# Artemarius/cuda-gaussian-splatting

Hardware: AMD Instinct MI355X
Metric: fwd+bwd Mpixels/s @1080p, 1M Gaussians, SH3 (higher is better)
Workload: dtype f32

## Files before the change

### cuda-gaussian-splatting_amd/csrc/cugs_raster_common.h

```cpp
#pragma once

#include "cugs_gaussian_math.h"

#define CUGS_REC_F4 3

struct RasterGeom {
    int width, height, ntx, ntiles;
    float bg0, bg1, bg2;
};

struct RasterSrc {
    const int32_t* tile_ranges;
    const int32_t* gidx;
    const float* packed;
    const float* means_2d;
    const float* cov_2d_inv;
    const float* rgb;
    const float* opa;
    const uint4* tile_order;
};

template <bool PACKED, bool DEPTH = false>
__device__ __forceinline__ int stage_record(const RasterSrc& s, int li, int end, float4* s_rec,
                                            const float* __restrict__ depths = nullptr) {
    if (li >= end) return -1;
    const int g = s.gidx[li];
    float4 r0, r1, r2;
    if (PACKED) {
        const float4* src = reinterpret_cast<const float4*>(s.packed + (int64_t)g * CUGS_PACKED_STRIDE);
        r0 = src[0]; r1 = src[1]; r2 = src[2];
    } else {
        const float a = s.cov_2d_inv[g * 3 + 0], c = s.cov_2d_inv[g * 3 + 2], o = s.opa[g];
        r0 = make_float4(s.means_2d[g * 2 + 0], s.means_2d[g * 2 + 1], a, s.cov_2d_inv[g * 3 + 1]);
        r1 = make_float4(c, o, (o >= (1.0f / 255.0f)) ? logf(255.0f * o) : -1.0f, 0.0f);
        r2 = make_float4(s.rgb[g * 3 + 0], 0.0f, s.rgb[g * 3 + 1], s.rgb[g * 3 + 2]);
    }
    r1.w = __int_as_float(g);
    if (DEPTH) r2.y = depths[g];
    s_rec[threadIdx.x * CUGS_REC_F4 + 0] = r0;
    s_rec[threadIdx.x * CUGS_REC_F4 + 1] = r1;
    s_rec[threadIdx.x * CUGS_REC_F4 + 2] = r2;
    return g;
}

__device__ __forceinline__ bool may_touch_quad(float4 r0, float4 r1, float qx0, float qy0,
                                               float wx, float wy) {
    const float mx = r0.x, my = r0.y, a = r0.z, b = r0.w, c = r1.x;
    const float tau = r1.z;
    if (!(tau >= 0.0f)) return false;
    if (!(a > 0.0f && c > 0.0f)) return true;
    const float ia = __builtin_amdgcn_rcpf(a), ic = __builtin_amdgcn_rcpf(c);
    const float lx = qx0 - mx, hx = lx + wx, ly = qy0 - my, hy = ly + wy;
    const bool inside = (lx <= 0.0f) && (hx >= 0.0f) && (ly <= 0.0f) && (hy >= 0.0f);
    float X, Y;
    asm("v_max_f32_e64 %0, -%1, %2" : "=v"(X) : "v"(lx), "v"(hx));
    asm("v_max_f32_e64 %0, -%1, %2" : "=v"(Y) : "v"(ly), "v"(hy));
    const float B = a * X * X + 2.0f * fabsf(b) * X * Y + c * Y * Y;
    const float b2 = b + b;
    const float xe = (lx > 0.0f) ? lx : hx, ye = (ly > 0.0f) ? ly : hy;
    const float yv = __builtin_amdgcn_fmed3f(-b * xe * ic, ly, hy);
    const float xv = __builtin_amdgcn_fmed3f(-b * ye * ia, lx, hx);
    const float qx = a * xe * xe + b2 * xe * yv + c * yv * yv;
    const float qy = a * xv * xv + b2 * xv * ye + c * ye * ye;
    const bool out_x = !((lx <= 0.0f) && (hx >= 0.0f)), out_y = !((ly <= 0.0f) && (hy >= 0.0f));
    const float qmin = inside ? 0.0f : fminf(out_x ? qx : 3.0e38f, out_y ? qy : 3.0e38f);
    return !(0.5f * qmin > tau * 1.01f + 0.05f + 4e-6f * B);
}

struct ActiveRect { float x0, y0, wx, wy; };
__device__ __forceinline__ ActiveRect active_rect(unsigned long long active, float quad_cx, float quad_cy) {
    unsigned cols = (unsigned)active | (unsigned)(active >> 32);
    cols |= cols >> 16;
    cols |= cols >> 8;
    cols &= 0xFFu;
    const int x0 = __builtin_ctz(cols), x1 = 31 - __builtin_clz(cols);
    const int y0 = __builtin_ctzll(active) >> 3, y1 = (63 - __builtin_clzll(active)) >> 3;
    return ActiveRect{quad_cx + (float)x0, quad_cy + (float)y0, (float)(x1 - x0), (float)(y1 - y0)};
}

#define CUGS_HIT_GROUP 4
__device__ __forceinline__ unsigned cugs_pop_hit_desc(unsigned long long& mask) {
    const unsigned bit = 63u - (unsigned)__builtin_clzll(mask);
    mask &= ~(1ull << bit);
    return bit;
}
__device__ __forceinline__ unsigned cugs_pop_hit_asc(unsigned long long& mask) {
    const unsigned bit = (unsigned)__builtin_ctzll(mask);
    mask &= mask - 1ull;
    return bit;
}
__device__ __forceinline__ unsigned long long cugs_pop_hits4_desc(unsigned long long& mask, unsigned rec_base) {
    const unsigned r0 = rec_base + cugs_pop_hit_desc(mask) * CUGS_REC_F4;
    const unsigned r1 = rec_base + cugs_pop_hit_desc(mask) * CUGS_REC_F4;
    const unsigned r2 = rec_base + cugs_pop_hit_desc(mask) * CUGS_REC_F4;
    const unsigned r3 = rec_base + cugs_pop_hit_desc(mask) * CUGS_REC_F4;
    return (unsigned long long)(r0 | (r1 << 16)) | ((unsigned long long)(r2 | (r3 << 16)) << 32);
}
__device__ __forceinline__ int cugs_hit(unsigned long long hitrecs, int field) {
    return (int)((hitrecs >> (16 * field)) & 0xFFFFull);
}
__device__ __forceinline__ unsigned long long cugs_set_hit(unsigned long long hitrecs, int field, unsigned rec) {
    return (hitrecs & ~(0xFFFFull << (16 * field))) | ((unsigned long long)rec << (16 * field));
}

struct PixelEval { float dx, dy, gx, gy, e; };
__device__ __forceinline__ float pixel_alpha_raw(float pxf, float pyf, float mx, float my, float a, float b,
                                                 float c, float o, float open, PixelEval& r) {
    r.dx = pxf - mx;
    r.dy = pyf - my;
    r.gx = fmaf(a, r.dx, b * r.dy);
    r.gy = fmaf(b, r.dx, c * r.dy);
    const float q = fmaf(r.dx, r.gx, r.dy * r.gy);
    r.e = cugs_blend_exp_q(q);
    const float gate = fmaf(q, 0x1p127f, 1.0f);
    return __builtin_fminf(__builtin_fminf((o * open) * r.e, 0.99f), gate);
}
__device__ __forceinline__ float pixel_alpha(float pxf, float pyf, float mx, float my, float a, float b,
                                             float c, float o, float open, PixelEval& r) {
    const float alpha = pixel_alpha_raw(pxf, pyf, mx, my, a, b, c, o, open, r);
    return (alpha < (1.0f / 255.0f)) ? 0.0f : alpha;
}


__device__ __forceinline__ float sat_fma(float a, float b, float c) {
    return __builtin_amdgcn_fmed3f(fmaf(a, b, c), 0.0f, 1.0f);
}
__device__ __forceinline__ float sat_add(float a, float b) { return __builtin_amdgcn_fmed3f(a + b, 0.0f, 1.0f); }

#define CUGS_ALPHA_MIN_PRED 0x1.01010p-8f
__device__ __forceinline__ float passes_alpha_min(float x) {
    return sat_fma(x, 0x1p32f, -CUGS_ALPHA_MIN_PRED * 0x1p32f);
}
__device__ __forceinline__ float below_alpha_cap(float x) { return sat_fma(x, -0x1p32f, 0.99f * 0x1p32f); }

__device__ __forceinline__ int reduce9t_slot(int lane) {
    if (lane & 3) return -1;
    const int bank = (lane >> 2) & 3, row = lane >> 4;
    const int perm[4] = {0, 2, 1, 3};
    if (row == 0) return perm[bank];
    if (row == 1) return bank == 3 ? 8 : 4 + perm[bank];
    if (row == 2 && bank == 0) return 7;
    return -1;
}

__device__ __forceinline__ float reduce9t(float cA, float cB, float v2, float v3, float v4, float v5, float v6,
                                          float v8, float v7) {
    float a0, a1, a2, a3, a4, b0, b1, b2, d;
    asm volatile(
// ... 126 lines not shown
```

### cuda-gaussian-splatting_amd/csrc/raster_backward.hip

```cpp
#include "cugs_raster_common.h"

#include <cstdlib>

#ifdef CUGS_DEV
bool cugs_dev_backward_stats();
#endif

namespace {

#define CUGS_BWD_HITS 4
static_assert(CUGS_BWD_HITS == CUGS_HIT_GROUP, "a hit group is one flush");
#ifndef CUGS_BWD_HSTRIDE
#define CUGS_BWD_HSTRIDE 64
#endif

template <bool PACKED, bool WIDE, bool STATS, bool DEPTH = false>
__global__ __launch_bounds__(CUGS_BLOCK) __attribute__((amdgpu_waves_per_eu(DEPTH ? 7 : 8)))
void k_raster_backward(RasterGeom geo, RasterSrc src,
                                                                const float* __restrict__ dL_dcolor,
                                                                const float* __restrict__ final_T,
                                                                const int32_t* __restrict__ n_contrib,
                                                                float* __restrict__ grad_accum, int64_t stats_row,
                                                                const float* __restrict__ depths,
                                                                const float* __restrict__ dL_ddepth_map,
                                                                const float* __restrict__ dL_dalpha) {
    __shared__ float4 s_rec[CUGS_BLOCK * CUGS_REC_F4];
    __shared__ float2 s_contrib[4][CUGS_BWD_HITS][CUGS_BWD_HSTRIDE];

#ifdef CUGS_DEV
    const bool no_atomics = stats_row == -2;
#else
    constexpr bool no_atomics = false;
#endif
    unsigned tile;
    int range_start, range_end;
    if (src.tile_order) {
        const uint4 rec = src.tile_order[blockIdx.x];
        tile = rec.x; range_start = (int)rec.y; range_end = (int)rec.z;
    } else {
        tile = cugs_blend_tile(blockIdx.x, (unsigned)geo.ntx, (unsigned)(geo.ntiles / geo.ntx));
        range_start = src.tile_ranges[tile * 2 + 0];
        range_end = src.tile_ranges[tile * 2 + 1];
    }
    const int tile_x = (int)(tile % (unsigned)geo.ntx), tile_y = (int)(tile / (unsigned)geo.ntx);
    const int tid = threadIdx.x, wave = tid >> 6, lane = tid & 63;
    const int quad_x = tile_x * CUGS_TILE + (wave & 1) * 8, quad_y = tile_y * CUGS_TILE + (wave >> 1) * 8;
    const int px = quad_x + (lane & 7), py = quad_y + (lane >> 3);
    const bool inside = (px < geo.width) && (py < geo.height);
    const float pxf = (float)px + 0.5f, pyf = (float)py + 0.5f;
    const float qx0 = (float)quad_x + 0.5f, qy0 = (float)quad_y + 0.5f;

    const int num_in_range = range_end - range_start;
    const int num_batches = (num_in_range + CUGS_BLOCK - 1) / CUGS_BLOCK;

    const int pix = py * geo.width + px;
    float T = inside ? final_T[pix] : 0.0f;
    const int max_contrib = inside ? n_contrib[pix] : 0;
    float dC0 = 0.0f, dC1 = 0.0f, dC2 = 0.0f;
    if (inside) {
        dC0 = dL_dcolor[pix * 3 + 0];
        dC1 = dL_dcolor[pix * 3 + 1];
        dC2 = dL_dcolor[pix * 3 + 2];
    }
    float dDp = 0.0f;
    if (DEPTH && inside && dL_ddepth_map) dDp = dL_ddepth_map[pix];
    const int h2 = lane >> 4, g2i = lane & 15;
    const int gx0 = quad_x + (g2i & 1) * 4, gy = quad_y + (g2i >> 1);
    const float px2 = (float)gx0 + 0.5f, py2 = (float)gy + 0.5f;
    const bool side = (lane & 8) != 0;
    float eA[4], eB[4], e2[4], eZ[4];
#pragma unroll
    for (int i = 0; i < 4; ++i) {
        float r = 0.0f, gg = 0.0f, bb = 0.0f, zz = 0.0f;
        if (gx0 + i < geo.width && gy < geo.height) {
            const int pq = gy * geo.width + gx0 + i, q = pq * 3;
            r = dL_dcolor[q + 0]; gg = dL_dcolor[q + 1]; bb = dL_dcolor[q + 2];
            if (DEPTH && dL_ddepth_map) zz = dL_ddepth_map[pq];
        }
        eA[i] = side ? gg : r; eB[i] = side ? r : gg; e2[i] = bb; eZ[i] = zz;
    }
    const int slot2 = DEPTH ? reduce10r16_slot(lane) : reduce9r16_slot(lane);
    const unsigned slot_off = (unsigned)(slot2 < 0 ? 0 : slot2) * 4u;
    unsigned long long hitrecs = 0ull;

    float D = fmaf(dC2, T * geo.bg2, fmaf(dC1, T * geo.bg1, dC0 * (T * geo.bg0)));
    if (DEPTH && inside && dL_dalpha) D = fmaf(-T, dL_dalpha[pix], D);
    float rem = (inside && max_contrib > 0) ? (float)max_contrib : -1.0f;
    float open = (inside && max_contrib > 0) ? 1.0f : 0.0f;
    bool wave_done = (__ballot(open != 0.0f) == 0ull);
    int pending = 0;
    unsigned st_steps = 0, st_contrib = 0, st_lanes = 0, st_batches = 0, st_tested = 0, st_open = 0;

    auto flush = [&](int cnt) {
        const int rec = (int)((hitrecs >> (16 * h2)) & 0xFFFFull);
        const float4* c4 = reinterpret_cast<const float4*>(&s_contrib[wave][h2][g2i * 4]);
        const float4 p01 = c4[0], p23 = c4[1];
        const float2 mean = *reinterpret_cast<const float2*>(&s_rec[rec]);
        const float4 tail = s_rec[rec + 1];
        const float dy = py2 - mean.y;
        const float dx0 = px2 - mean.x, dx1 = dx0 + 1.0f, dx2 = dx0 + 2.0f, dx3 = dx0 + 3.0f;
        float t = p01.y * dx0;
        float A = p01.y, M1 = t, Mxx = t * dx0;
        float RA = p01.x * eA[0], RB = p01.x * eB[0], R2 = p01.x * e2[0];
        t = p01.w * dx1; A += p01.w; M1 += t; Mxx = fmaf(t, dx1, Mxx);
        RA = fmaf(p01.z, eA[1], RA); RB = fmaf(p01.z, eB[1], RB); R2 = fmaf(p01.z, e2[1], R2);
        t = p23.y * dx2; A += p23.y; M1 += t; Mxx = fmaf(t, dx2, Mxx);
        RA = fmaf(p23.x, eA[2], RA); RB = fmaf(p23.x, eB[2], RB); R2 = fmaf(p23.x, e2[2], R2);
        t = p23.w * dx3; A += p23.w; M1 += t; Mxx = fmaf(t, dx3, Mxx);
        RA = fmaf(p23.z, eA[3], RA); RB = fmaf(p23.z, eB[3], RB); R2 = fmaf(p23.z, e2[3], R2);
        const float oA = tail.y * A;
        M1 *= tail.y; Mxx *= tail.y;
        const float M1y = dy * oA, Myy = dy * M1y, Mxy = dy * M1;
        float total;
        if (DEPTH) {
            float RZ = p01.x * eZ[0];
            RZ = fmaf(p01.z, eZ[1], RZ); RZ = fmaf(p23.x, eZ[2], RZ); RZ = fmaf(p23.z, eZ[3], RZ);
            total = reduce10r16(RA, RB, R2, A, M1, M1y, Mxx, Myy, Mxy, RZ, lane);
        } else {
            total = reduce9r16(RA, RB, R2, A, M1, M1y, Mxx, Myy, Mxy, lane);
        }
        if (slot2 >= 0 && h2 < cnt && !no_atomics) {
            const int g = __float_as_int(tail.w);
            if (WIDE) {
                atomicAdd(grad_accum + (int64_t)g * CUGS_GRAD_STRIDE + slot2, total);
            } else {
                const unsigned off = ((unsigned)g << 6) + slot_off;
                atomicAdd(reinterpret_cast<float*>(reinterpret_cast<char*>(grad_accum) + off), total);
            }
        }
    };

    auto step = [&](const int rec, const int slot) __attribute__((always_inline)) {
        if (STATS) ++st_steps;
        const float4 g0 = s_rec[rec], g1 = s_rec[rec + 1], col = s_rec[rec + 2];
        const float o = g1.y;

        PixelEval e;
        const float alpha = pixel_alpha_raw(pxf, pyf, g0.x, g0.y, g0.z, g0.w, g1.x, o, open, e);
        const float passf = passes_alpha_min(alpha);
        rem -= passf;
        open = sat_add(rem, 1.0f);
        const float k = passf * open;
        const float al = alpha * k;
        const float gk = k * below_alpha_cap(alpha);

        const float rcp = __builtin_amdgcn_rcpf(1.0f - al);
        T *= rcp;
        const float weight = al * T;
        float G = fmaf(dC2, col.w, fmaf(dC1, col.z, dC0 * col.x));
        if (DEPTH) G = fmaf(dDp, col.y, G);
        const float gate = fmaf(T, G, -(rcp * D)) * gk;
        D = fmaf(weight, G, D);
        if (STATS) {
            const unsigned long long lm = __ballot(k != 0.0f);
            if (lm) { ++st_contrib; st_lanes += __popcll(lm); st_open += __popcll(__ballot(open != 0.0f)); }
        }
        s_contrib[wave][slot][lane] = make_float2(weight, gate * e.e);
    };

    for (int batch = num_batches - 1; batch >= 0; --batch) {
        if (lane == 0) s_contrib[wave][0][0].x = wave_done ? 1.0f : 0.0f;
        __syncthreads();
        if (s_contrib[0][0][0].x * s_contrib[1][0][0].x * s_contrib[2][0][0].x * s_contrib[3][0][0].x != 0.0f) break;

        stage_record<PACKED, DEPTH>(src, range_start + batch * CUGS_BLOCK + tid, range_end, s_rec, depths);
        __syncthreads();

        if (STATS && !wave_done) ++st_batches;
        if (!wave_done) {
            const int batch_count = min(CUGS_BLOCK, num_in_range - batch * CUGS_BLOCK);
            const int nsub = (batch_count + CUGS_WAVE - 1) / CUGS_WAVE;
            for (int sub = nsub - 1; sub >= 0 && !wave_done; --sub) {
                const int j = sub * CUGS_WAVE + lane;
                const ActiveRect ar = active_rect(__ballot(open != 0.0f), qx0, qy0);
                bool hit = false;
                if (j < batch_count)
                    hit = may_touch_quad(s_rec[j * CUGS_REC_F4 + 0], s_rec[j * CUGS_REC_F4 + 1], ar.x0, ar.y0, ar.wx,
                                         ar.wy);
                unsigned long long mask = __ballot(hit);
                if (STATS) st_tested += min(CUGS_WAVE, batch_count - sub * CUGS_WAVE);
                const unsigned rec_sub = (unsigned)(sub * CUGS_WAVE * CUGS_REC_F4);
                while (pending + __popcll(mask) >= CUGS_BWD_HITS) {
                    if (pending == 0) {
                        hitrecs = cugs_pop_hits4_desc(mask, rec_sub);
                    } else {
                        do hitrecs = cugs_set_hit(hitrecs, pending, rec_sub + cugs_pop_hit_desc(mask) * CUGS_REC_F4);
                        while (++pending < CUGS_BWD_HITS);
                        pending = 0;
                    }
                    step(cugs_hit(hitrecs, 0), 0);
                    step(cugs_hit(hitrecs, 1), 1);
                    step(cugs_hit(hitrecs, 2), 2);
                    step(cugs_hit(hitrecs, 3), 3);
                    const bool closed = (__ballot(open != 0.0f) == 0ull);
                    flush(CUGS_BWD_HITS);
                    if (closed) { wave_done = true; mask = 0ull; break; }
                }
                while (mask != 0ull) {
                    hitrecs = cugs_set_hit(hitrecs, pending, rec_sub + cugs_pop_hit_desc(mask) * CUGS_REC_F4);
                    ++pending;
                }
            }
            if (pending) {
                for (int p = 0; p < pending; ++p) step(cugs_hit(hitrecs, p), p);
                if (__ballot(open != 0.0f) == 0ull) wave_done = true;
                flush(pending);
                pending = 0;
            }
        }
    }
    if (STATS && lane == 0) {
        float* st = grad_accum + (int64_t)stats_row * CUGS_GRAD_STRIDE;
        atomicAdd(&st[0], (float)st_steps); atomicAdd(&st[1], (float)st_contrib); atomicAdd(&st[2], (float)st_lanes);
        atomicAdd(&st[3], (float)st_batches); atomicAdd(&st[4], (float)st_tested); atomicAdd(&st[5], (float)num_batches);
        atomicAdd(&st[7], (float)st_open);
    }
}

template <bool PACKED, bool DEPTH = false>
__global__ __launch_bounds__(CUGS_BLOCK) void k_unpack_grads(int64_t n, const float* __restrict__ acc,
                                                             const float* __restrict__ packed,
                                                             const float* __restrict__ cov_2d_inv,
                                                             float* __restrict__ dL_drgb,
                                                             float* __restrict__ dL_dopa,
                                                             float* __restrict__ dL_dmeans,
                                                             float* __restrict__ dL_dcov,
                                                             float* __restrict__ dL_ddepths) {
    const int64_t i = (int64_t)blockIdx.x * CUGS_BLOCK + threadIdx.x;
    if (i >= n) return;
    const float4* row = reinterpret_cast<const float4*>(acc + i * CUGS_GRAD_STRIDE);
    const float4 r0 = row[0], r1 = row[1];
    float r2;
    if (DEPTH) {
        const float2 w89 = *reinterpret_cast<const float2*>(acc + i * CUGS_GRAD_STRIDE + 8);
        r2 = w89.x;
        dL_ddepths[i] = w89.y;
    } else {
        r2 = acc[i * CUGS_GRAD_STRIDE + 8];
    }
    float a, b, c;
    if (PACKED) {
        const float4* rec = reinterpret_cast<const float4*>(packed + i * CUGS_PACKED_STRIDE);
        const float4 p0 = rec[0];
        a = p0.z; b = p0.w; c = rec[1].x;
    } else {
        a = cov_2d_inv[i * 3 + 0]; b = cov_2d_inv[i * 3 + 1]; c = cov_2d_inv[i * 3 + 2];
    }
    dL_drgb[i * 3 + 0] = r0.x; dL_drgb[i * 3 + 1] = r0.y; dL_drgb[i * 3 + 2] = r0.z;
    dL_dopa[i] = r0.w;
    const GradMoments m{r1.x, r1.y, r1.z, r1.w, r2};
    const Grad2D g = grads_from_moments(m, a, b, c);
    dL_dmeans[i * 2 + 0] = g.mx; dL_dmeans[i * 2 + 1] = g.my;
    dL_dcov[i * 3 + 0] = g.a; dL_dcov[i * 3 + 1] = g.b; dL_dcov[i * 3 + 2] = g.c;
}

}

namespace {
int rasterize_backward_impl(int width, int height, const float background_host[3],
                                       const int32_t* tile_ranges, const int32_t* gaussian_indices,
                                       const float* means_2d, const float* cov_2d_inv, const float* rgb,
                                       const float* opacities_act, const float* packed,
                                       const float* dL_dcolor, const float* final_T,
                                       const int32_t* n_contrib, int64_t n, float* grad_accum,
                                       float* dL_drgb, float* dL_dopacity_act, float* dL_dmeans_2d,
                                       float* dL_dcov_2d_inv, bool prezeroed, const uint32_t* tile_order, void* stream,
                                       bool depth_map = false, const float* depths = nullptr,
                                       const float* dL_ddepth_map = nullptr, const float* dL_dalpha = nullptr,
// ... 142 lines not shown
                      in[6 * 64 + l], in[8 * 64 + l], in[7 * 64 + l]);
    slots[l] = reduce9t_slot(l);
}
__global__ void k_dbg_reduce9r16(const float* __restrict__ in, float* __restrict__ out, int* __restrict__ slots) {
    const int l = threadIdx.x;
    const bool side = (l & 8) != 0;
    const float v0 = in[0 * 64 + l], v1 = in[1 * 64 + l];
    out[l] = reduce9r16(side ? v1 : v0, side ? v0 : v1, in[2 * 64 + l], in[3 * 64 + l], in[4 * 64 + l], in[5 * 64 + l],
                        in[6 * 64 + l], in[8 * 64 + l], in[7 * 64 + l], l);
    slots[l] = reduce9r16_slot(l);
}
__global__ void k_dbg_reduce10r16(const float* __restrict__ in, float* __restrict__ out, int* __restrict__ slots) {
    const int l = threadIdx.x;
    const bool side = (l & 8) != 0;
    const float v0 = in[0 * 64 + l], v1 = in[1 * 64 + l];
    out[l] = reduce10r16(side ? v1 : v0, side ? v0 : v1, in[2 * 64 + l], in[3 * 64 + l], in[4 * 64 + l], in[5 * 64 + l],
                         in[6 * 64 + l], in[8 * 64 + l], in[7 * 64 + l], in[9 * 64 + l], l);
    slots[l] = reduce10r16_slot(l);
}
__global__ void k_dbg_rcp(const float* __restrict__ in, float* __restrict__ out, int n) {
    const int i = blockIdx.x * blockDim.x + threadIdx.x;
    if (i < n) out[i] = __builtin_amdgcn_rcpf(in[i]);
}
__global__ void k_dbg_blend_exp(const float* __restrict__ q, float* __restrict__ out, int n) {
    const int i = blockIdx.x * blockDim.x + threadIdx.x;
    if (i < n) out[i] = cugs_blend_exp_q(q[i]);
}
__global__ void k_dbg_may_touch_quad(int n, const float* __restrict__ in, const unsigned long long* __restrict__ masks,
                                     int* __restrict__ hit, unsigned long long* __restrict__ pass,
                                     float* __restrict__ rect) {
    const int i = blockIdx.x * blockDim.x + threadIdx.x;
    if (i >= n) return;
    const float* c = in + (int64_t)i * 8;
    alignas(16) float rec[CUGS_PACKED_STRIDE];
    write_packed(rec, 0, c[0], c[1], Sym2{c[2], c[3], c[4]}, 0.0f, 0.0f, 0.0f, c[5]);
    const float4 r0 = reinterpret_cast<const float4*>(rec)[0], r1 = reinterpret_cast<const float4*>(rec)[1];
    const int quad_x = (int)c[6], quad_y = (int)c[7];
    const float qx0 = (float)quad_x + 0.5f, qy0 = (float)quad_y + 0.5f;
    const unsigned long long active = masks[i];
    const ActiveRect ar = active_rect(active, qx0, qy0);
    hit[i] = may_touch_quad(r0, r1, ar.x0, ar.y0, ar.wx, ar.wy) ? 1 : 0;
    unsigned long long p = 0ull;
    for (int l = 0; l < 64; ++l) {
        const float pxf = (float)(quad_x + (l & 7)) + 0.5f, pyf = (float)(quad_y + (l >> 3)) + 0.5f;
        const float open = ((active >> l) & 1ull) ? 1.0f : 0.0f;
        PixelEval e;
        const float alpha = pixel_alpha_raw(pxf, pyf, r0.x, r0.y, r0.z, r0.w, r1.x, r1.y, open, e);
        if (passes_alpha_min(alpha) != 0.0f) p |= 1ull << l;
    }
    pass[i] = p;
    rect[(int64_t)i * 4 + 0] = ar.x0 - qx0; rect[(int64_t)i * 4 + 1] = ar.y0 - qy0;
    rect[(int64_t)i * 4 + 2] = ar.wx; rect[(int64_t)i * 4 + 3] = ar.wy;
}
bool g_dev_backward_stats = false;
}
bool cugs_dev_backward_stats() { return g_dev_backward_stats; }
extern "C" int cugsdbg_backward_stats(int on) { g_dev_backward_stats = (on != 0); return 0; }
extern "C" int cugsdbg_reduce9(const float* in, float* out, int* slots, void* stream) {
    hipLaunchKernelGGL(k_dbg_reduce9, dim3(1), dim3(64), 0, static_cast<hipStream_t>(stream), in, out, slots);
    CUGS_LAUNCH_CHECK();
    return 0;
}
extern "C" int cugsdbg_reduce9r16(const float* in, float* out, int* slots, void* stream) {
    hipLaunchKernelGGL(k_dbg_reduce9r16, dim3(1), dim3(64), 0, static_cast<hipStream_t>(stream), in, out, slots);
    CUGS_LAUNCH_CHECK();
    return 0;
}
extern "C" int cugsdbg_reduce10r16(const float* in, float* out, int* slots, void* stream) {
    hipLaunchKernelGGL(k_dbg_reduce10r16, dim3(1), dim3(64), 0, static_cast<hipStream_t>(stream), in, out, slots);
    CUGS_LAUNCH_CHECK();
    return 0;
}
extern "C" int cugsdbg_blend_exp_q(const float* q, float* out, int n, void* stream) {
    hipLaunchKernelGGL(k_dbg_blend_exp, dim3((n + 255) / 256), dim3(256), 0, static_cast<hipStream_t>(stream), q, out, n);
    CUGS_LAUNCH_CHECK();
    return 0;
}
extern "C" int cugsdbg_rcp(const float* in, float* out, int n, void* stream) {
    hipLaunchKernelGGL(k_dbg_rcp, dim3((n + 255) / 256), dim3(256), 0, static_cast<hipStream_t>(stream), in, out, n);
    CUGS_LAUNCH_CHECK();
    return 0;
}
extern "C" int cugsdbg_may_touch_quad(int n, const float* in, const unsigned long long* masks, int* hit,
                                      unsigned long long* pass, float* rect, void* stream) {
    if (n <= 0) return n == 0 ? 0 : CUGS_EINVAL;
    hipLaunchKernelGGL(k_dbg_may_touch_quad, dim3((n + 255) / 256), dim3(256), 0, static_cast<hipStream_t>(stream), n, in,
                       masks, hit, pass, rect);
    CUGS_LAUNCH_CHECK();
    return 0;
}
#endif
```

### cuda-gaussian-splatting_amd/csrc/raster_forward.hip

```cpp
#include "cugs_raster_common.h"

namespace {

template <bool PACKED, bool DEPTH>
__device__ __forceinline__ void raster_forward_tile(RasterGeom geo, RasterSrc src, float* out_color, float* out_final_T,
                                                    int32_t* out_n_contrib, float4* zero_buf, uint32_t zero_vec4,
                                                    const float* depths, float* out_depth) {
    __shared__ float4 s_rec[CUGS_BLOCK * CUGS_REC_F4];
    __shared__ int s_wave_done[4];

    if (zero_buf) {
        const uint32_t per = (zero_vec4 + gridDim.x - 1) / gridDim.x;
        const uint32_t lo = blockIdx.x * per, hi = min(zero_vec4, lo + per);
        for (uint32_t e = lo + threadIdx.x; e < hi; e += CUGS_BLOCK) cugs_stnt(zero_buf + e, make_float4(0.0f, 0.0f, 0.0f, 0.0f));
    }

    unsigned tile;
    int range_start, range_end;
    if (src.tile_order) {
        const uint4 rec = src.tile_order[blockIdx.x];
        tile = rec.x; range_start = (int)rec.y; range_end = (int)rec.z;
    } else {
        tile = cugs_blend_tile(blockIdx.x, (unsigned)geo.ntx, (unsigned)(geo.ntiles / geo.ntx));
        range_start = src.tile_ranges[tile * 2 + 0];
        range_end = src.tile_ranges[tile * 2 + 1];
    }
    const int tile_x = (int)(tile % (unsigned)geo.ntx), tile_y = (int)(tile / (unsigned)geo.ntx);
    const int tid = threadIdx.x, wave = tid >> 6, lane = tid & 63;
    const int quad_x = tile_x * CUGS_TILE + (wave & 1) * 8, quad_y = tile_y * CUGS_TILE + (wave >> 1) * 8;
    const int px = quad_x + (lane & 7), py = quad_y + (lane >> 3);
    const bool inside = (px < geo.width) && (py < geo.height);
    const float pxf = (float)px + 0.5f, pyf = (float)py + 0.5f;
    const float qx0 = (float)quad_x + 0.5f, qy0 = (float)quad_y + 0.5f;

    const int num_in_range = range_end - range_start;
    const int num_batches = (num_in_range + CUGS_BLOCK - 1) / CUGS_BLOCK;

    typedef float v2f __attribute__((ext_vector_type(2)));
    float T = 1.0f, C0 = 0.0f;
    v2f C12 = {0.0f, 0.0f};
    v2f C0Z = {0.0f, 0.0f};
    float count = 0.0f;
    float open = inside ? 1.0f : 0.0f;
    bool wave_done = (__ballot(open != 0.0f) == 0ull);

    auto step = [&](const float4* rp) __attribute__((always_inline)) {
        const float4 g0 = rp[0], g1 = rp[1], col = rp[2];
        const float o = g1.y;
        PixelEval e;
        const float alpha = pixel_alpha_raw(pxf, pyf, g0.x, g0.y, g0.z, g0.w, g1.x, o, open, e);
        const float passf = passes_alpha_min(alpha);
        const float al = alpha * passf;
        const float weight = al * T;
        if (DEPTH) C0Z = __builtin_elementwise_fma((v2f){weight, weight}, (v2f){col.x, col.y}, C0Z);
        else C0 = fmaf(weight, col.x, C0);
        C12 = __builtin_elementwise_fma((v2f){weight, weight}, (v2f){col.z, col.w}, C12);
        T *= (1.0f - al);
        count += passf;
        open *= passes_alpha_min(T);
    };

    for (int batch = 0; batch < num_batches; ++batch) {
        if (lane == 0) s_wave_done[wave] = wave_done ? 1 : 0;
        __syncthreads();
        if (s_wave_done[0] & s_wave_done[1] & s_wave_done[2] & s_wave_done[3]) break;

        stage_record<PACKED, DEPTH>(src, range_start + batch * CUGS_BLOCK + tid, range_end, s_rec, depths);
        __syncthreads();

        if (!wave_done) {
            const int batch_count = min(CUGS_BLOCK, num_in_range - batch * CUGS_BLOCK);
            for (int sub = 0; sub * CUGS_WAVE < batch_count && !wave_done; ++sub) {
                const int j = sub * CUGS_WAVE + lane;
                const ActiveRect ar = active_rect(__ballot(open != 0.0f), qx0, qy0);
                bool hit = false;
                if (j < batch_count)
                    hit = may_touch_quad(s_rec[j * CUGS_REC_F4 + 0], s_rec[j * CUGS_REC_F4 + 1], ar.x0, ar.y0, ar.wx,
                                         ar.wy);
                unsigned long long mask = __ballot(hit);
                const float4* sub_rec = s_rec + sub * CUGS_WAVE * CUGS_REC_F4;
                while (__popcll(mask) >= CUGS_HIT_GROUP) {
                    const float4* r0 = sub_rec + cugs_pop_hit_asc(mask) * CUGS_REC_F4;
                    const float4* r1 = sub_rec + cugs_pop_hit_asc(mask) * CUGS_REC_F4;
                    const float4* r2 = sub_rec + cugs_pop_hit_asc(mask) * CUGS_REC_F4;
                    const float4* r3 = sub_rec + cugs_pop_hit_asc(mask) * CUGS_REC_F4;
                    step(r0); step(r1); step(r2); step(r3);
                    if (__ballot(open != 0.0f) == 0ull) { wave_done = true; mask = 0ull; break; }
                }
                while (mask != 0ull) {
                    step(sub_rec + cugs_pop_hit_asc(mask) * CUGS_REC_F4);
                    if (__ballot(open != 0.0f) == 0ull) { wave_done = true; break; }
                }
            }
        }
    }

    if (inside) {
        const int pix = py * geo.width + px;
        if (DEPTH) {
            C0 = C0Z.x;
            out_depth[pix] = fmaf(T, 0.0f, C0Z.y);
        }
        out_color[pix * 3 + 0] = fmaf(T, geo.bg0, C0);
        out_color[pix * 3 + 1] = fmaf(T, geo.bg1, C12.x);
        out_color[pix * 3 + 2] = fmaf(T, geo.bg2, C12.y);
        out_final_T[pix] = T;
        out_n_contrib[pix] = (int)count;
    }
}

template <bool PACKED>
__global__ __launch_bounds__(CUGS_BLOCK) void k_raster_forward(RasterGeom geo, RasterSrc src,
                                                               float* __restrict__ out_color,
                                                               float* __restrict__ out_final_T,
                                                               int32_t* __restrict__ out_n_contrib,
                                                               float4* __restrict__ zero_buf, uint32_t zero_vec4) {
    raster_forward_tile<PACKED, false>(geo, src, out_color, out_final_T, out_n_contrib, zero_buf, zero_vec4, nullptr,
                                       nullptr);
}

template <bool PACKED>
__global__ __launch_bounds__(CUGS_BLOCK) void k_raster_forward_depth(RasterGeom geo, RasterSrc src,
                                                                     float* __restrict__ out_color,
                                                                     float* __restrict__ out_final_T,
                                                                     int32_t* __restrict__ out_n_contrib,
                                                                     float4* __restrict__ zero_buf, uint32_t zero_vec4,
                                                                     const float* __restrict__ depths,
                                                                     float* __restrict__ out_depth) {
    raster_forward_tile<PACKED, true>(geo, src, out_color, out_final_T, out_n_contrib, zero_buf, zero_vec4, depths,
                                      out_depth);
}

}

namespace {
int rasterize_forward_impl(int width, int height, const float background_host[3], const int32_t* tile_ranges,
                           const int32_t* gaussian_indices, const float* means_2d, const float* cov_2d_inv,
                           const float* rgb, const float* opacities_act, const float* packed, float* out_color,
                           float* out_final_T, int32_t* out_n_contrib, void* zero_buf, size_t zero_bytes,
                           const uint32_t* tile_order, void* stream, bool depth_map = false,
                           const float* depths = nullptr, float* out_depth = nullptr) {
    if (width < 0 || height < 0 || !background_host) return CUGS_EINVAL;
    if (zero_bytes && (!zero_buf || (reinterpret_cast<uintptr_t>(zero_buf) & 15u) || (zero_bytes & 15u) ||
                       zero_bytes / 16 > 0xFFFFFFFFull))
        return zero_buf ? CUGS_EALIGN : CUGS_EINVAL;
    const int ntx = (width + CUGS_TILE - 1) / CUGS_TILE, nty = (height + CUGS_TILE - 1) / CUGS_TILE;
    if (ntx == 0 || nty == 0) {
        if (zero_bytes) CUGS_RETURN_IF_HIP(hipMemsetAsync(zero_buf, 0, zero_bytes, static_cast<hipStream_t>(stream)));
        return 0;
// ... 19 lines not shown
    } else if (packed) {
        hipLaunchKernelGGL((k_raster_forward<true>), dim3(geo.ntiles), dim3(CUGS_BLOCK), 0, st, geo, src,
                           out_color, out_final_T, out_n_contrib, zb, zv);
    } else {
        hipLaunchKernelGGL((k_raster_forward<false>), dim3(geo.ntiles), dim3(CUGS_BLOCK), 0, st, geo, src,
                           out_color, out_final_T, out_n_contrib, zb, zv);
    }
    CUGS_LAUNCH_CHECK();
    return 0;
}
}

extern "C" int cugs_rasterize_forward(int width, int height, const float background_host[3],
                                      const int32_t* tile_ranges, const int32_t* gaussian_indices,
                                      const float* means_2d, const float* cov_2d_inv, const float* rgb,
                                      const float* opacities_act, const float* packed, float* out_color,
                                      float* out_final_T, int32_t* out_n_contrib, void* stream) {
    return rasterize_forward_impl(width, height, background_host, tile_ranges, gaussian_indices, means_2d, cov_2d_inv, rgb,
                                  opacities_act, packed, out_color, out_final_T, out_n_contrib, nullptr, 0, nullptr, stream);
}

extern "C" int cugs_rasterize_forward_zero(int width, int height, const float background_host[3],
                                           const int32_t* tile_ranges, const int32_t* gaussian_indices,
                                           const float* means_2d, const float* cov_2d_inv, const float* rgb,
                                           const float* opacities_act, const float* packed, float* out_color,
                                           float* out_final_T, int32_t* out_n_contrib, void* zero_buf,
                                           size_t zero_bytes, void* stream) {
    return rasterize_forward_impl(width, height, background_host, tile_ranges, gaussian_indices, means_2d, cov_2d_inv, rgb,
                                  opacities_act, packed, out_color, out_final_T, out_n_contrib, zero_buf, zero_bytes, nullptr, stream);
}

extern "C" int cugs_rasterize_forward_ordered(int width, int height, const float background_host[3],
                                              const int32_t* tile_ranges, const int32_t* gaussian_indices,
                                              const float* means_2d, const float* cov_2d_inv, const float* rgb,
                                              const float* opacities_act, const float* packed, float* out_color,
                                              float* out_final_T, int32_t* out_n_contrib, void* zero_buf,
                                              size_t zero_bytes, const uint32_t* tile_order, void* stream) {
    return rasterize_forward_impl(width, height, background_host, tile_ranges, gaussian_indices, means_2d, cov_2d_inv, rgb,
                                  opacities_act, packed, out_color, out_final_T, out_n_contrib, zero_buf, zero_bytes, tile_order,
                                  stream);
}

extern "C" int cugs_rasterize_forward_depth(int width, int height, const float background_host[3],
                                            const int32_t* tile_ranges, const int32_t* gaussian_indices,
                                            const float* means_2d, const float* cov_2d_inv, const float* rgb,
                                            const float* opacities_act, const float* packed, float* out_color,
                                            float* out_final_T, int32_t* out_n_contrib, void* zero_buf,
                                            size_t zero_bytes, const uint32_t* tile_order, const float* depths,
                                            float* out_depth, void* stream) {
    return rasterize_forward_impl(width, height, background_host, tile_ranges, gaussian_indices, means_2d, cov_2d_inv, rgb,
                                  opacities_act, packed, out_color, out_final_T, out_n_contrib, zero_buf, zero_bytes, tile_order,
                                  stream, true, depths, out_depth);
}
```

Baseline: 2705.

## Merge disjoint-coverage Gaussian pairs into single evaluation step in backward raster

While staging records, the backward kernel now computes a per-tile row/column coverage bitmask for each Gaussian and stores it in a spare record field. Two consecutive hits whose masks do not overlap within the wave's 8x8 quad are treated as twins. Each lane evaluates only the Gaussian that covers it and writes zero contributions for the other slot, so one eval replaces two. The cost is extra work per staged record, a bpermute and ballot per sub-batch, and more branching, and it only runs in the non-depth path.

```diff
diff --git a/cuda-gaussian-splatting_amd/csrc/cugs_raster_common.h b/cuda-gaussian-splatting_amd/csrc/cugs_raster_common.h
--- a/cuda-gaussian-splatting_amd/csrc/cugs_raster_common.h
+++ b/cuda-gaussian-splatting_amd/csrc/cugs_raster_common.h
@@ -20,9 +20,11 @@
     const uint4* tile_order;
 };
 
-template <bool PACKED, bool DEPTH = false>
+__device__ __forceinline__ unsigned cugs_tile_cover(float4 r0, float4 r1, float tcx0, float tcy0);
+template <bool PACKED, bool DEPTH = false, bool COVER = false>
 __device__ __forceinline__ int stage_record(const RasterSrc& s, int li, int end, float4* s_rec,
-                                            const float* __restrict__ depths = nullptr) {
+                                            const float* __restrict__ depths = nullptr, float tcx0 = 0.0f,
+                                            float tcy0 = 0.0f) {
     if (li >= end) return -1;
     const int g = s.gidx[li];
     float4 r0, r1, r2;
@@ -37,6 +39,7 @@
     }
     r1.w = __int_as_float(g);
     if (DEPTH) r2.y = depths[g];
+    if (COVER && !DEPTH) r2.y = __uint_as_float(cugs_tile_cover(r0, r1, tcx0, tcy0));
     s_rec[threadIdx.x * CUGS_REC_F4 + 0] = r0;
     s_rec[threadIdx.x * CUGS_REC_F4 + 1] = r1;
     s_rec[threadIdx.x * CUGS_REC_F4 + 2] = r2;
@@ -78,6 +81,50 @@
     return ActiveRect{quad_cx + (float)x0, quad_cy + (float)y0, (float)(x1 - x0), (float)(y1 - y0)};
 }
 
+#define CUGS_COVER_FULL 0xFFFFFFFFu
+__device__ __forceinline__ unsigned cugs_cover_bits(float lo, float ext) {
+    const float f0 = fminf(fmaxf(ceilf(-lo - ext), 0.0f), 16.0f), f1 = fminf(fmaxf(floorf(ext - lo), -1.0f), 15.0f);
+    if (!(f0 <= f1)) return (lo != lo || ext != ext) ? 0xFFFFu : 0u;
+    return (2u << (unsigned)(int)f1) - (1u << (unsigned)(int)f0);
+}
+__device__ __forceinline__ unsigned cugs_tile_cover(float4 r0, float4 r1, float tcx0, float tcy0) {
+    const float mx = r0.x, my = r0.y, a = r0.z, b = r0.w, c = r1.x, tau = r1.z;
+    const float ac = a * c, det = ac - b * b;
+    if (!(tau >= 0.0f && a > 0.0f && c > 0.0f && det > ac * 0x1p-10f)) return CUGS_COVER_FULL;
+    const float lx = tcx0 - mx, ly = tcy0 - my;
+    const float X = fmaxf(-lx, lx + 15.0f), Y = fmaxf(-ly, ly + 15.0f);
+    const float B = a * X * X + 2.0f * fabsf(b) * X * Y + c * Y * Y;
+    const float r = 2.0f * (tau * 1.01f + 0.05f + 4e-6f * B) / det;
+    return cugs_cover_bits(lx, sqrtf(r * c)) | (cugs_cover_bits(ly, sqrtf(r * a)) << 16);
+}
+__device__ __forceinline__ unsigned cugs_quad_cover(int wave) {
+    return (0xFFu << (8 * (wave & 1))) | (0xFF0000u << (8 * (wave >> 1)));
+}
+__device__ __forceinline__ bool cugs_covers_meet(unsigned cov_a, unsigned cov_b, unsigned quad) {
+    const unsigned t = cov_a & cov_b & quad;
+    return (t & 0xFFFFu) != 0u && (t >> 16) != 0u;
+}
+__device__ __forceinline__ unsigned long long cugs_cover_lanes(unsigned cov, int wave) {
+    const unsigned cols = (cov >> (8 * (wave & 1))) & 0xFFu, rows = (cov >> (16 + 8 * (wave >> 1))) & 0xFFu;
+    if (rows == 0u) return 0ull;
+    const unsigned y0 = (unsigned)__builtin_ctz(rows), n = (unsigned)__builtin_popcount(rows);
+    const unsigned long long run = (n >= 8u) ? ~0ull : (((1ull << (8u * n)) - 1ull) << (8u * y0));
+    const unsigned c4 = cols * 0x01010101u;
+    return run & (((unsigned long long)c4 << 32) | c4);
+}
+__device__ __forceinline__ int cugs_select_lanes(int a, int b, unsigned long long m) {
+    int r;
+    asm("v_cndmask_b32_e64 %0, %1, %2, %3" : "=v"(r) : "v"(a), "v"(b), "s"(m));
+    return r;
+}
+__device__ __forceinline__ unsigned long long cugs_twin_mask(unsigned long long mask, bool hit, unsigned cov,
+                                                              unsigned quad, int lane) {
+    const unsigned long long above = (mask >> 1) >> lane;
+    const int prev = (lane + 1 + __builtin_ctzll(above | (1ull << 63))) & 63;
+    const unsigned pc = (unsigned)__builtin_amdgcn_ds_bpermute(prev << 2, (int)cov);
+    return __ballot(hit && above != 0ull && !cugs_covers_meet(cov, pc, quad));
+}
+
 #define CUGS_HIT_GROUP 4
 __device__ __forceinline__ unsigned cugs_pop_hit_desc(unsigned long long& mask) {
     const unsigned bit = 63u - (unsigned)__builtin_clzll(mask);
@@ -94,6 +141,16 @@
     const unsigned r1 = rec_base + cugs_pop_hit_desc(mask) * CUGS_REC_F4;
     const unsigned r2 = rec_base + cugs_pop_hit_desc(mask) * CUGS_REC_F4;
     const unsigned r3 = rec_base + cugs_pop_hit_desc(mask) * CUGS_REC_F4;
+    return (unsigned long long)(r0 | (r1 << 16)) | ((unsigned long long)(r2 | (r3 << 16)) << 32);
+}
+__device__ __forceinline__ unsigned long long cugs_pop_hits4_desc_twins(unsigned long long& mask, unsigned rec_base,
+                                                                        unsigned long long twins, unsigned& tw) {
+    const unsigned b0 = cugs_pop_hit_desc(mask), b1 = cugs_pop_hit_desc(mask), b2 = cugs_pop_hit_desc(mask),
+                   b3 = cugs_pop_hit_desc(mask);
+    tw = (unsigned)((twins >> b1) & 1ull) | ((unsigned)((twins >> b2) & 1ull) << 1) |
+         ((unsigned)((twins >> b3) & 1ull) << 2);
+    const unsigned r0 = rec_base + b0 * CUGS_REC_F4, r1 = rec_base + b1 * CUGS_REC_F4;
+    const unsigned r2 = rec_base + b2 * CUGS_REC_F4, r3 = rec_base + b3 * CUGS_REC_F4;
     return (unsigned long long)(r0 | (r1 << 16)) | ((unsigned long long)(r2 | (r3 << 16)) << 32);
 }
 __device__ __forceinline__ int cugs_hit(unsigned long long hitrecs, int field) {
diff --git a/cuda-gaussian-splatting_amd/csrc/raster_backward.hip b/cuda-gaussian-splatting_amd/csrc/raster_backward.hip
--- a/cuda-gaussian-splatting_amd/csrc/raster_backward.hip
+++ b/cuda-gaussian-splatting_amd/csrc/raster_backward.hip
@@ -26,6 +26,7 @@
                                                                 const float* __restrict__ dL_dalpha) {
     __shared__ float4 s_rec[CUGS_BLOCK * CUGS_REC_F4];
     __shared__ float2 s_contrib[4][CUGS_BWD_HITS][CUGS_BWD_HSTRIDE];
+    constexpr bool TWIN = !DEPTH;
 
 #ifdef CUGS_DEV
     const bool no_atomics = stats_row == -2;
@@ -49,6 +50,9 @@
     const bool inside = (px < geo.width) && (py < geo.height);
     const float pxf = (float)px + 0.5f, pyf = (float)py + 0.5f;
     const float qx0 = (float)quad_x + 0.5f, qy0 = (float)quad_y + 0.5f;
+    const float tcx0 = (float)(tile_x * CUGS_TILE) + 0.5f, tcy0 = (float)(tile_y * CUGS_TILE) + 0.5f;
+    const int wave_s = __builtin_amdgcn_readfirstlane(wave);
+    const unsigned quad_cover = cugs_quad_cover(wave_s);
 
     const int num_in_range = range_end - range_start;
     const int num_batches = (num_in_range + CUGS_BLOCK - 1) / CUGS_BLOCK;
@@ -89,7 +93,7 @@
     float open = (inside && max_contrib > 0) ? 1.0f : 0.0f;
     bool wave_done = (__ballot(open != 0.0f) == 0ull);
     int pending = 0;
-    unsigned st_steps = 0, st_contrib = 0, st_lanes = 0, st_batches = 0, st_tested = 0, st_open = 0;
+    unsigned st_steps = 0, st_contrib = 0, st_lanes = 0, st_batches = 0, st_tested = 0, st_open = 0, st_twins = 0;
 
     auto flush = [&](int cnt) {
         const int rec = (int)((hitrecs >> (16 * h2)) & 0xFFFFull);
@@ -130,9 +134,8 @@
         }
     };
 
-    auto step = [&](const int rec, const int slot) __attribute__((always_inline)) {
+    auto eval = [&](const float4 g0, const float4 g1, const float4 col) __attribute__((always_inline)) {
         if (STATS) ++st_steps;
-        const float4 g0 = s_rec[rec], g1 = s_rec[rec + 1], col = s_rec[rec + 2];
         const float o = g1.y;
 
         PixelEval e;
@@ -155,7 +158,20 @@
             const unsigned long long lm = __ballot(k != 0.0f);
             if (lm) { ++st_contrib; st_lanes += __popcll(lm); st_open += __popcll(__ballot(open != 0.0f)); }
         }
-        s_contrib[wave][slot][lane] = make_float2(weight, gate * e.e);
+        return make_float2(weight, gate * e.e);
+    };
+    auto step = [&](const int rec, const int slot) __attribute__((always_inline)) {
+        s_contrib[wave][slot][lane] = eval(s_rec[rec], s_rec[rec + 1], s_rec[rec + 2]);
+    };
+    auto twin = [&](const int rec_a, const int rec_b, const int slot_a, const int slot_b) __attribute__((always_inline)) {
+        if (STATS) ++st_twins;
+        const unsigned cov_b = (unsigned)__builtin_amdgcn_readfirstlane((int)__float_as_uint(s_rec[rec_b + 2].y));
+        const unsigned long long in_b = cugs_cover_lanes(cov_b, wave_s);
+        const int rec = cugs_select_lanes(rec_a, rec_b, in_b);
+        const float2 v = eval(s_rec[rec], s_rec[rec + 1], s_rec[rec + 2]);
+        const int slot = cugs_select_lanes(slot_a, slot_b, in_b);
+        s_contrib[wave][slot][lane] = v;
+        s_contrib[wave][slot_a + slot_b - slot][lane] = make_float2(0.0f, 0.0f);
     };
 
     for (int batch = num_batches - 1; batch >= 0; --batch) {
@@ -163,7 +179,7 @@
         __syncthreads();
         if (s_contrib[0][0][0].x * s_contrib[1][0][0].x * s_contrib[2][0][0].x * s_contrib[3][0][0].x != 0.0f) break;
 
-        stage_record<PACKED, DEPTH>(src, range_start + batch * CUGS_BLOCK + tid, range_end, s_rec, depths);
+        stage_record<PACKED, DEPTH, TWIN>(src, range_start + batch * CUGS_BLOCK + tid, range_end, s_rec, depths, tcx0, tcy0);
         __syncthreads();
 
         if (STATS && !wave_done) ++st_batches;
@@ -180,18 +196,35 @@
                 unsigned long long mask = __ballot(hit);
                 if (STATS) st_tested += min(CUGS_WAVE, batch_count - sub * CUGS_WAVE);
                 const unsigned rec_sub = (unsigned)(sub * CUGS_WAVE * CUGS_REC_F4);
+                unsigned long long twins = 0ull;
+                if (TWIN && pending + __popcll(mask) >= CUGS_BWD_HITS)
+                    twins = cugs_twin_mask(mask, hit, __float_as_uint(s_rec[(j & (CUGS_BLOCK - 1)) * CUGS_REC_F4 + 2].y),
+                                           quad_cover, lane);
                 while (pending + __popcll(mask) >= CUGS_BWD_HITS) {
+                    unsigned tw = 0u;
                     if (pending == 0) {
-                        hitrecs = cugs_pop_hits4_desc(mask, rec_sub);
+                        if (TWIN) hitrecs = cugs_pop_hits4_desc_twins(mask, rec_sub, twins, tw);
+                        else hitrecs = cugs_pop_hits4_desc(mask, rec_sub);
                     } else {
                         do hitrecs = cugs_set_hit(hitrecs, pending, rec_sub + cugs_pop_hit_desc(mask) * CUGS_REC_F4);
                         while (++pending < CUGS_BWD_HITS);
                         pending = 0;
                     }
-                    step(cugs_hit(hitrecs, 0), 0);
-                    step(cugs_hit(hitrecs, 1), 1);
-                    step(cugs_hit(hitrecs, 2), 2);
-                    step(cugs_hit(hitrecs, 3), 3);
+                    if (!TWIN || tw == 0u) {
+                        step(cugs_hit(hitrecs, 0), 0);
+                        step(cugs_hit(hitrecs, 1), 1);
+                        step(cugs_hit(hitrecs, 2), 2);
+                        step(cugs_hit(hitrecs, 3), 3);
+                    } else if ((tw & 5u) == 0u) {
+                        step(cugs_hit(hitrecs, 0), 0);
+                        twin(cugs_hit(hitrecs, 1), cugs_hit(hitrecs, 2), 1, 2);
+                        step(cugs_hit(hitrecs, 3), 3);
+                    } else {
+                        if (tw & 1u) twin(cugs_hit(hitrecs, 0), cugs_hit(hitrecs, 1), 0, 1);
+                        else { step(cugs_hit(hitrecs, 0), 0); step(cugs_hit(hitrecs, 1), 1); }
+                        if (tw & 4u) twin(cugs_hit(hitrecs, 2), cugs_hit(hitrecs, 3), 2, 3);
+                        else { step(cugs_hit(hitrecs, 2), 2); step(cugs_hit(hitrecs, 3), 3); }
+                    }
                     const bool closed = (__ballot(open != 0.0f) == 0ull);
                     flush(CUGS_BWD_HITS);
                     if (closed) { wave_done = true; mask = 0ull; break; }
@@ -213,7 +246,7 @@
         float* st = grad_accum + (int64_t)stats_row * CUGS_GRAD_STRIDE;
         atomicAdd(&st[0], (float)st_steps); atomicAdd(&st[1], (float)st_contrib); atomicAdd(&st[2], (float)st_lanes);
         atomicAdd(&st[3], (float)st_batches); atomicAdd(&st[4], (float)st_tested); atomicAdd(&st[5], (float)num_batches);
-        atomicAdd(&st[7], (float)st_open);
+        atomicAdd(&st[6], (float)st_twins); atomicAdd(&st[7], (float)st_open);
     }
 }
 
```

Measured after the change: 2606. -3.7%, worse.

## Precompute per-quad cull bits at staging time in forward rasterizer

Applied to the files above, without the earlier changes.

During record staging, each thread now evaluates the Gaussian against all four 8x8 quads of the tile once and packs the four hit bits into the high bits of the index word. Waves whose active pixel area is large enough then read their bit instead of running the per-wave ellipse-vs-rectangle test for every record and sub-batch. Quads already marked done are skipped in the static test. This moves redundant culling work from four waves to a single staging pass. The cost is extra arithmetic during staging, coarser culling when many pixels are active, and a limit of 28 bits on Gaussian indices.

```diff
diff --git a/cuda-gaussian-splatting_amd/csrc/cugs_raster_common.h b/cuda-gaussian-splatting_amd/csrc/cugs_raster_common.h
--- a/cuda-gaussian-splatting_amd/csrc/cugs_raster_common.h
+++ b/cuda-gaussian-splatting_amd/csrc/cugs_raster_common.h
@@ -19,29 +19,6 @@
     const float* opa;
     const uint4* tile_order;
 };
-
-template <bool PACKED, bool DEPTH = false>
-__device__ __forceinline__ int stage_record(const RasterSrc& s, int li, int end, float4* s_rec,
-                                            const float* __restrict__ depths = nullptr) {
-    if (li >= end) return -1;
-    const int g = s.gidx[li];
-    float4 r0, r1, r2;
-    if (PACKED) {
-        const float4* src = reinterpret_cast<const float4*>(s.packed + (int64_t)g * CUGS_PACKED_STRIDE);
-        r0 = src[0]; r1 = src[1]; r2 = src[2];
-    } else {
-        const float a = s.cov_2d_inv[g * 3 + 0], c = s.cov_2d_inv[g * 3 + 2], o = s.opa[g];
-        r0 = make_float4(s.means_2d[g * 2 + 0], s.means_2d[g * 2 + 1], a, s.cov_2d_inv[g * 3 + 1]);
-        r1 = make_float4(c, o, (o >= (1.0f / 255.0f)) ? logf(255.0f * o) : -1.0f, 0.0f);
-        r2 = make_float4(s.rgb[g * 3 + 0], 0.0f, s.rgb[g * 3 + 1], s.rgb[g * 3 + 2]);
-    }
-    r1.w = __int_as_float(g);
-    if (DEPTH) r2.y = depths[g];
-    s_rec[threadIdx.x * CUGS_REC_F4 + 0] = r0;
-    s_rec[threadIdx.x * CUGS_REC_F4 + 1] = r1;
-    s_rec[threadIdx.x * CUGS_REC_F4 + 2] = r2;
-    return g;
-}
 
 __device__ __forceinline__ bool may_touch_quad(float4 r0, float4 r1, float qx0, float qy0,
                                                float wx, float wy) {
@@ -78,6 +55,119 @@
     return ActiveRect{quad_cx + (float)x0, quad_cy + (float)y0, (float)(x1 - x0), (float)(y1 - y0)};
 }
 
+#define CUGS_QUAD_BITS_SHIFT 28
+#define CUGS_REC_INDEX_MASK ((1u << CUGS_QUAD_BITS_SHIFT) - 1u)
+
+struct QuadCullAxis {
+    float l, h;
+    float E2;
+    float E;
+    float bE;
+    float e;
+    float v;
+    float e2;
+    float be;
+    bool in;
+};
+__device__ __forceinline__ QuadCullAxis quad_cull_axis(float q0, float m, float d, float id, float nb, float ab2,
+                                                       float b2) {
+    QuadCullAxis r;
+    r.l = q0 - m;
+    r.h = r.l + 7.0f;
+    r.in = (r.l <= 0.0f) && (r.h >= 0.0f);
+    asm("v_max_f32_e64 %0, -%1, %2" : "=v"(r.E) : "v"(r.l), "v"(r.h));
+    r.E2 = d * r.E * r.E;
+    r.bE = ab2 * r.E;
+    r.e = (r.l > 0.0f) ? r.l : r.h;
+    r.v = nb * r.e * id;
+    r.e2 = d * r.e * r.e;
+    r.be = b2 * r.e;
+    return r;
+}
+__device__ __forceinline__ bool quad_cull_one(const QuadCullAxis& cx, const QuadCullAxis& cy, float a, float c, float b2,
+                                              float thr) {
+    const bool inside = cx.in && cy.in;
+    const float B = cx.E2 + cx.bE * cy.E + cy.E2;
+    const float yv = __builtin_amdgcn_fmed3f(cx.v, cy.l, cy.h);
+    const float xv = __builtin_amdgcn_fmed3f(cy.v, cx.l, cx.h);
+    const float qx = cx.e2 + cx.be * yv + c * yv * yv;
+    const float qy = a * xv * xv + b2 * xv * cy.e + cy.e2;
+    const float qmin = inside ? 0.0f : fminf(!cx.in ? qx : 3.0e38f, !cy.in ? qy : 3.0e38f);
+    return !(0.5f * qmin > thr + 4e-6f * B);
+}
+__device__ __forceinline__ unsigned static_quad_bits(float4 r0, float4 r1, int tile_px, int tile_py, unsigned skip) {
+    const float mx = r0.x, my = r0.y, a = r0.z, b = r0.w, c = r1.x;
+    const float tau = r1.z;
+    if (!(tau >= 0.0f)) return 0u;
+    if (!(a > 0.0f && c > 0.0f)) return 0xFu;
+    const float ia = __builtin_amdgcn_rcpf(a), ic = __builtin_amdgcn_rcpf(c);
+    const float b2 = b + b, ab2 = 2.0f * fabsf(b), nb = -b;
+    const float thr = tau * 1.01f + 0.05f;
+    const QuadCullAxis x0 = quad_cull_axis((float)tile_px + 0.5f, mx, a, ic, nb, ab2, b2);
+    const QuadCullAxis x1 = quad_cull_axis((float)(tile_px + 8) + 0.5f, mx, a, ic, nb, ab2, b2);
+    unsigned bits = 0u;
+    if ((skip & 3u) != 3u) {
+        const QuadCullAxis y0 = quad_cull_axis((float)tile_py + 0.5f, my, c, ia, nb, ab2, b2);
+        if (!(skip & 1u) && quad_cull_one(x0, y0, a, c, b2, thr)) bits |= 1u;
+        if (!(skip & 2u) && quad_cull_one(x1, y0, a, c, b2, thr)) bits |= 2u;
+    }
+    if ((skip & 12u) != 12u) {
+        const QuadCullAxis y1 = quad_cull_axis((float)(tile_py + 8) + 0.5f, my, c, ia, nb, ab2, b2);
+        if (!(skip & 4u) && quad_cull_one(x0, y1, a, c, b2, thr)) bits |= 4u;
+        if (!(skip & 8u) && quad_cull_one(x1, y1, a, c, b2, thr)) bits |= 8u;
+    }
+    return bits;
+}
+
+__device__ __forceinline__ int active_area(unsigned long long active) {
+    unsigned cols = (unsigned)active | (unsigned)(active >> 32);
+    cols |= cols >> 16;
+    cols |= cols >> 8;
+    cols &= 0xFFu;
+    const int x0 = __builtin_ctz(cols), x1 = 31 - __builtin_clz(cols);
+    const int y0 = __builtin_ctzll(active) >> 3, y1 = (63 - __builtin_clzll(active)) >> 3;
+    return (x1 - x0 + 1) * (y1 - y0 + 1);
+}
+template <int MIN_AREA>
+__device__ __forceinline__ bool use_static_bits(unsigned long long active) {
+    if (MIN_AREA <= 1 || __popcll(active) >= MIN_AREA) return true;
+    if (MIN_AREA > 64) return false;
+    return active_area(active) >= MIN_AREA;
+}
+__device__ __forceinline__ bool static_hit(const float4* s_rec, int j, int wave) {
+    const unsigned w7 = __float_as_uint(s_rec[j * CUGS_REC_F4 + 1].w);
+    return ((w7 >> (CUGS_QUAD_BITS_SHIFT + wave)) & 1u) != 0u;
+}
+
+template <bool PACKED, bool DEPTH = false, bool QUAD_BITS = false>
+__device__ __forceinline__ int stage_record(const RasterSrc& s, int li, int end, float4* s_rec,
+                                            const float* __restrict__ depths = nullptr, int tile_px = 0, int tile_py = 0,
+                                            unsigned skip = 0u) {
+    if (li >= end) return -1;
+    const int g = s.gidx[li];
+    float4 r0, r1, r2;
+    if (PACKED) {
+        const float4* src = reinterpret_cast<const float4*>(s.packed + (int64_t)g * CUGS_PACKED_STRIDE);
+        r0 = src[0]; r1 = src[1]; r2 = src[2];
+    } else {
+        const float a = s.cov_2d_inv[g * 3 + 0], c = s.cov_2d_inv[g * 3 + 2], o = s.opa[g];
+        r0 = make_float4(s.means_2d[g * 2 + 0], s.means_2d[g * 2 + 1], a, s.cov_2d_inv[g * 3 + 1]);
+        r1 = make_float4(c, o, (o >= (1.0f / 255.0f)) ? logf(255.0f * o) : -1.0f, 0.0f);
+        r2 = make_float4(s.rgb[g * 3 + 0], 0.0f, s.rgb[g * 3 + 1], s.rgb[g * 3 + 2]);
+    }
+    r1.w = __int_as_float(g);
+    if (DEPTH) r2.y = depths[g];
+    s_rec[threadIdx.x * CUGS_REC_F4 + 0] = r0;
+    s_rec[threadIdx.x * CUGS_REC_F4 + 1] = r1;
+    s_rec[threadIdx.x * CUGS_REC_F4 + 2] = r2;
+    if (QUAD_BITS) {
+        const unsigned bits = static_quad_bits(r0, r1, tile_px, tile_py, skip);
+        s_rec[threadIdx.x * CUGS_REC_F4 + 1].w =
+            __uint_as_float(((unsigned)g & CUGS_REC_INDEX_MASK) | (bits << CUGS_QUAD_BITS_SHIFT));
+    }
+    return g;
+}
+
 #define CUGS_HIT_GROUP 4
 __device__ __forceinline__ unsigned cugs_pop_hit_desc(unsigned long long& mask) {
     const unsigned bit = 63u - (unsigned)__builtin_clzll(mask);
diff --git a/cuda-gaussian-splatting_amd/csrc/raster_backward.hip b/cuda-gaussian-splatting_amd/csrc/raster_backward.hip
--- a/cuda-gaussian-splatting_amd/csrc/raster_backward.hip
+++ b/cuda-gaussian-splatting_amd/csrc/raster_backward.hip
@@ -462,6 +462,15 @@
     rect[(int64_t)i * 4 + 0] = ar.x0 - qx0; rect[(int64_t)i * 4 + 1] = ar.y0 - qy0;
     rect[(int64_t)i * 4 + 2] = ar.wx; rect[(int64_t)i * 4 + 3] = ar.wy;
 }
+__global__ void k_dbg_static_quad_bits(int n, const float* __restrict__ in, int* __restrict__ bits) {
+    const int i = blockIdx.x * blockDim.x + threadIdx.x;
+    if (i >= n) return;
+    const float* c = in + (int64_t)i * 8;
+    alignas(16) float rec[CUGS_PACKED_STRIDE];
+    write_packed(rec, 0, c[0], c[1], Sym2{c[2], c[3], c[4]}, 0.0f, 0.0f, 0.0f, c[5]);
+    const float4 r0 = reinterpret_cast<const float4*>(rec)[0], r1 = reinterpret_cast<const float4*>(rec)[1];
+    bits[i] = (int)static_quad_bits(r0, r1, (int)c[6], (int)c[7], 0u);
+}
 bool g_dev_backward_stats = false;
 }
 bool cugs_dev_backward_stats() { return g_dev_backward_stats; }
@@ -499,4 +508,11 @@
     CUGS_LAUNCH_CHECK();
     return 0;
 }
-#endif
+extern "C" int cugsdbg_static_quad_bits(int n, const float* in, int* bits, void* stream) {
+    if (n <= 0) return n == 0 ? 0 : CUGS_EINVAL;
+    hipLaunchKernelGGL(k_dbg_static_quad_bits, dim3((n + 255) / 256), dim3(256), 0, static_cast<hipStream_t>(stream), n, in,
+                       bits);
+    CUGS_LAUNCH_CHECK();
+    return 0;
+}
+#endif
diff --git a/cuda-gaussian-splatting_amd/csrc/raster_forward.hip b/cuda-gaussian-splatting_amd/csrc/raster_forward.hip
--- a/cuda-gaussian-splatting_amd/csrc/raster_forward.hip
+++ b/cuda-gaussian-splatting_amd/csrc/raster_forward.hip
@@ -1,4 +1,16 @@
 #include "cugs_raster_common.h"
+
+#ifndef CUGS_FWD_STATIC_MIN_AREA
+#define CUGS_FWD_STATIC_MIN_AREA 16
+#endif
+
+#ifdef CUGS_DEV
+__device__ unsigned long long g_fwd_stats[3];
+__device__ int g_fwd_stats_on;
+#define CUGS_FWD_COUNT(x) do { x; } while (0)
+#else
+#define CUGS_FWD_COUNT(x) do { } while (0)
+#endif
 
 namespace {
 
@@ -43,8 +55,10 @@
     float count = 0.0f;
     float open = inside ? 1.0f : 0.0f;
     bool wave_done = (__ballot(open != 0.0f) == 0ull);
+    [[maybe_unused]] unsigned st_steps = 0, st_tests = 0, st_bits = 0;
 
     auto step = [&](const float4* rp) __attribute__((always_inline)) {
+        CUGS_FWD_COUNT(++st_steps);
         const float4 g0 = rp[0], g1 = rp[1], col = rp[2];
         const float o = g1.y;
         PixelEval e;
@@ -63,20 +77,30 @@
     for (int batch = 0; batch < num_batches; ++batch) {
         if (lane == 0) s_wave_done[wave] = wave_done ? 1 : 0;
         __syncthreads();
-        if (s_wave_done[0] & s_wave_done[1] & s_wave_done[2] & s_wave_done[3]) break;
-
-        stage_record<PACKED, DEPTH>(src, range_start + batch * CUGS_BLOCK + tid, range_end, s_rec, depths);
+        const unsigned done_quads = __builtin_amdgcn_readfirstlane(
+            (unsigned)(s_wave_done[0] | (s_wave_done[1] << 1) | (s_wave_done[2] << 2) | (s_wave_done[3] << 3)));
+        if (done_quads == 0xFu) break;
+
+        stage_record<PACKED, DEPTH, true>(src, range_start + batch * CUGS_BLOCK + tid, range_end, s_rec, depths,
+                                          tile_x * CUGS_TILE, tile_y * CUGS_TILE, done_quads);
         __syncthreads();
 
         if (!wave_done) {
             const int batch_count = min(CUGS_BLOCK, num_in_range - batch * CUGS_BLOCK);
             for (int sub = 0; sub * CUGS_WAVE < batch_count && !wave_done; ++sub) {
                 const int j = sub * CUGS_WAVE + lane;
-                const ActiveRect ar = active_rect(__ballot(open != 0.0f), qx0, qy0);
+                const unsigned long long active = __ballot(open != 0.0f);
                 bool hit = false;
-                if (j < batch_count)
-                    hit = may_touch_quad(s_rec[j * CUGS_REC_F4 + 0], s_rec[j * CUGS_REC_F4 + 1], ar.x0, ar.y0, ar.wx,
-                                         ar.wy);
+                if (use_static_bits<CUGS_FWD_STATIC_MIN_AREA>(active)) {
+                    if (j < batch_count) hit = static_hit(s_rec, j, wave);
+                    CUGS_FWD_COUNT(st_bits += min(CUGS_WAVE, batch_count - sub * CUGS_WAVE));
+                } else {
+                    const ActiveRect ar = active_rect(active, qx0, qy0);
+                    if (j < batch_count)
+                        hit = may_touch_quad(s_rec[j * CUGS_REC_F4 + 0], s_rec[j * CUGS_REC_F4 + 1], ar.x0, ar.y0, ar.wx,
+                                             ar.wy);
+                    CUGS_FWD_COUNT(st_tests += min(CUGS_WAVE, batch_count - sub * CUGS_WAVE));
+                }
                 unsigned long long mask = __ballot(hit);
                 const float4* sub_rec = s_rec + sub * CUGS_WAVE * CUGS_REC_F4;
                 while (__popcll(mask) >= CUGS_HIT_GROUP) {
@@ -95,6 +119,13 @@
         }
     }
 
+#ifdef CUGS_DEV
+    if (lane == 0 && g_fwd_stats_on) {
+        atomicAdd(&g_fwd_stats[0], (unsigned long long)st_steps);
+        atomicAdd(&g_fwd_stats[1], (unsigned long long)st_tests);
+        atomicAdd(&g_fwd_stats[2], (unsigned long long)st_bits);
+    }
+#endif
     if (inside) {
         const int pix = py * geo.width + px;
         if (DEPTH) {
@@ -220,3 +251,15 @@
                                   opacities_act, packed, out_color, out_final_T, out_n_contrib, zero_buf, zero_bytes, tile_order,
                                   stream, true, depths, out_depth);
 }
+
+#ifdef CUGS_DEV
+extern "C" int cugsdbg_forward_stats(int on, unsigned long long* out3) {
+    const unsigned long long zero[3] = {0ull, 0ull, 0ull};
+    const int flag = on ? 1 : 0;
+    CUGS_RETURN_IF_HIP(hipDeviceSynchronize());
+    if (on) CUGS_RETURN_IF_HIP(hipMemcpyToSymbol(HIP_SYMBOL(g_fwd_stats), zero, sizeof(zero)));
+    else if (out3) CUGS_RETURN_IF_HIP(hipMemcpyFromSymbol(out3, HIP_SYMBOL(g_fwd_stats), sizeof(zero)));
+    CUGS_RETURN_IF_HIP(hipMemcpyToSymbol(HIP_SYMBOL(g_fwd_stats_on), &flag, sizeof(flag)));
+    return 0;
+}
+#endif
```

Result: no change. 2700 before, 2700 after (median of 2 runs) (+0.0%).
